# zhangzhousuper/Radish_PT

Hardware: AMD Instinct MI355X
Metric: Mrays/s (higher is better)
Workload: dtype f32

## Files before the change

### radish_pt_amd/_build.py

```python
import os
import subprocess
import sys

ROOT = os.path.dirname(os.path.dirname(os.path.abspath(__file__)))
CSRC = os.path.join(ROOT, "radish_pt_amd", "csrc")
HIPCC = os.environ.get("HIPCC", "/opt/rocm/bin/hipcc")

HOST_SOURCES = [os.path.join(CSRC, "host", "scene_build.cpp"), os.path.join(CSRC, "host", "scene_load.cpp")]
HIP_SOURCES = [os.path.join(CSRC, "radish_hip.hip")]
HIP_DEPS = [
    os.path.join(CSRC, "device", f)
    for f in ("rmath.h", "layouts.h", "traverse.h", "bsdf.h", "lights.h", "path_step.h", "kernels_pt.h", "kernels_restir.h", "kernels_wave.h", "kernels_persist.h", "kernels_walk.h", "wg_trace.h", "kernels_display.h", "kernels_denoise.h", "kernels_bvh.h", "kernels_refit.h", "kernels_lbvh.h", "kernels_lights.h", "kernels_pose.h", "kernels_materials.h", "kernels_textures.h")
] + [os.path.join(ROOT, "include", "radish_hip.h")]

HIP_FLAGS = [
    "--offload-arch=gfx950", "-O3", "-std=c++17", "-fPIC", "-shared", "-ffp-contract=off", "-fno-fast-math",
    "-fno-gpu-rdc", "-Wall", "-Wno-unused-function", "-Wno-unused-value", "-Wno-unused-result",
]


def _newer(target, deps):
    if not os.path.exists(target):
        return True
    t = os.path.getmtime(target)
    return any(os.path.exists(d) and os.path.getmtime(d) > t for d in deps)


def _run(cmd):
    print("[build]", " ".join(cmd), flush=True)
    subprocess.check_call(cmd)


def build_host(force=False):
    out = os.path.join(CSRC, "libradish_host.so")
    deps = HOST_SOURCES + [os.path.join(ROOT, "include", "radish_host.h")]
    if force or _newer(out, deps):
        _run(["g++", "-O2", "-std=c++17", "-fPIC", "-shared", "-ffp-contract=off", "-fno-fast-math", "-Wall", "-o", out]
             + HOST_SOURCES + ["-lz"])
    return out


def build_hip(force=False):
    out = os.path.join(CSRC, "libradish_hip.so")
    if force or _newer(out, HIP_SOURCES + HIP_DEPS):
        _run([HIPCC] + HIP_FLAGS + ["-I", os.path.join(ROOT, "include"), "-o", out] + HIP_SOURCES
             + ["-Wl,-rpath,/opt/rocm/lib"])
    return out


def build_variant(name, defines):
    d = os.path.join(CSRC, "variants")
    os.makedirs(d, exist_ok=True)
    out = os.path.join(d, f"libradish_hip_{name}.so")
    _run([HIPCC] + HIP_FLAGS + [f"-D{x}" for x in defines] + ["-I", os.path.join(ROOT, "include"), "-o", out]
         + HIP_SOURCES + ["-Wl,-rpath,/opt/rocm/lib"])
    return out


def build_all(force=False):
    build_host(force)
    build_hip(force)


if __name__ == "__main__":
    build_all(force="--force" in sys.argv)
```

### radish_pt_amd/csrc/device/kernels_wave.h

```cpp
#pragma once
#include "kernels_pt.h"
#include "wg_trace.h"

namespace rd {

constexpr int kWfLitCap = 8192;
constexpr int kWfLitShadow = 0x40000000;
constexpr int kMaxWaveDepth = 32;

struct alignas(128) WaveCounter {
    int v;
    int pad[31];
};
#ifndef RD_WF_TICKET_SHARDS
#define RD_WF_TICKET_SHARDS 8
#endif
constexpr int kTicketShards = RD_WF_TICKET_SHARDS;
struct WaveCounters {
    WaveCounter rayCount[kMaxWaveDepth + 2];
    WaveCounter shadowCount[kMaxWaveDepth + 2];
    WaveCounter litCount[kMaxWaveDepth + 2];
    WaveCounter traceHead[kMaxWaveDepth + 2];
    WaveCounter shadeHead[kMaxWaveDepth + 2][4];
    WaveCounter traceTicket[kMaxWaveDepth + 2][kTicketShards];
    WaveCounter shadeTicket[kMaxWaveDepth + 2][kTicketShards];
};

struct WaveWorkspace {
    float4 *ro[2];
    float4 *rd[2];
    float4 *thr[2];
    float4 *prevPos[2];
    float4 *accD;
    float4 *accI;
    float4 *nee[2];
    float4 *sht[2];
    uint2 *rng[2];
    int4 *hit;
    int *rayq[2];
    int *shadowq;
    int *litq[2];
    int litCap;
    int *treeOvf;
    int treeOvfDepth;
#ifdef RD_WF_STAMPS
    unsigned long long *stamps;
    int stampWaves;
#endif
    WaveCounters *ctr;
};

constexpr unsigned kWfNeeNone = 2u;
RD_DEV float wfNeeTag(int home, unsigned kind) { return __uint_as_float(((unsigned)home << 2) | kind); }
RD_DEV void wfAddNee(const WaveWorkspace &w, float4 n) {
    const unsigned tag = __float_as_uint(n.w), kind = tag & 3u;
    if (kind == kWfNeeNone) return;
    float4 *acc = (kind == 0u ? w.accD : w.accI) + (tag >> 2);
    const float4 a = *acc;
    *acc = make_float4(a.x + n.x, a.y + n.y, a.z + n.z, 0.f);
}

RD_DEV Ray wfSlotRay(const WaveWorkspace &w, int set, int p, bool shadow, float &limit) {
    if (shadow) {
        const float4 x = w.prevPos[set][p], y = w.sht[set][p];
        return shadowRay(mk3(x.x, x.y, x.z), mk3(y.x, y.y, y.z), limit);
    }
    const float4 o = w.ro[set][p], d = w.rd[set][p];
    limit = 3.402823466e+38f;
    return Ray{mk3(o.x, o.y, o.z), mk3(d.x, d.y, d.z)};
}

struct WaveSlotPath {
    const WaveWorkspace &w;
    const int rs, p;
    const int wr, q;
    int home;
    const bool delta;
    RD_DEV v3 throughput() {
        const float4 t = w.thr[rs][p];
        home = __float_as_int(t.w);
        return mk3(t.x, t.y, t.z);
    }
    RD_DEV float samplePdf() const { return w.ro[rs][p].w; }
    RD_DEV bool sampleDelta() const { return delta; }
    RD_DEV v3 prevPos() const { const float4 c = w.prevPos[rs][p]; return mk3(c.x, c.y, c.z); }
    RD_DEV void setDirect(v3 v) { w.accD[home] = make_float4(v.x, v.y, v.z, 0.f); }
    RD_DEV void addIndirect(v3 v) { const float4 a = w.accI[home]; w.accI[home] = make_float4(a.x + v.x, a.y + v.y, a.z + v.z, 0.f); }
    RD_DEV Sampler rng(const DScene &s) const { const uint2 r = w.rng[rs][p]; return Sampler{s.sobol, r.x, (int)r.y}; }
    RD_DEV void setNee(v3 c, float nw) { w.nee[wr][q] = make_float4(c.x, c.y, c.z, wfNeeTag(home, nw < 0.f ? kWfNeeNone : (nw == 0.f ? 0u : 1u))); }
    RD_DEV void setPrevPos(v3 x) { w.prevPos[wr][q] = make_float4(x.x, x.y, x.z, 0.f); }
    RD_DEV void setRay(const Ray &ray, float pdf, bool deltaSample, v3 throughput, const Sampler &rng) {
        w.ro[wr][q] = make_float4(ray.o.x, ray.o.y, ray.o.z, pdf);
        w.rd[wr][q] = make_float4(ray.d.x, ray.d.y, ray.d.z, deltaSample ? 1.f : 0.f);
        w.thr[wr][q] = make_float4(throughput.x, throughput.y, throughput.z, __int_as_float(home));
        w.rng[wr][q] = make_uint2(rng.scramble, (unsigned)rng.ptr);
    }
};


RD_DEV void waveAppend(bool pred, int item, int *queue, int *count) {
    unsigned long long mask = __ballot(pred);
    if (mask == 0ull) return;
    int leader = __ffsll((long long)mask) - 1;
    int base = 0;
    if ((int)(threadIdx.x & 63u) == leader) base = atomicAdd(count, __popcll(mask));
    base = __shfl(base, leader, 64);
    if (pred) queue[base + __popcll(mask & laneMaskLt())] = item;
}

constexpr int kShadeChunks = 4;
constexpr int kShadePacket = 64 * kShadeChunks;
RD_DEV void waveAppendN(const bool (&pred)[kShadeChunks], const int (&item)[kShadeChunks], int *queue, int *count) {
    unsigned long long m[kShadeChunks];
    int total = 0;
#pragma unroll
    for (int j = 0; j < kShadeChunks; j++) {
        m[j] = __ballot(pred[j]);
        total += __popcll(m[j]);
    }
    if (total == 0) return;
    int base = 0;
    if ((threadIdx.x & 63u) == 0u) base = atomicAdd(count, total);
    base = __shfl(base, 0, 64);
#pragma unroll
    for (int j = 0; j < kShadeChunks; j++) {
        if (pred[j]) queue[base + __popcll(m[j] & laneMaskLt())] = item[j];
        base += __popcll(m[j]);
    }
}

constexpr int kPacket = 128;
RD_DEV int gridWaves() { return int(gridDim.x * (blockDim.x >> 6)); }
RD_DEV int workgroupTicket(WaveCounter *tickets) {
    __shared__ int ticket;
    if (threadIdx.x == 0) {
        const unsigned x = blockIdx.x % (unsigned)kTicketShards;
        ticket = int(x + (unsigned)kTicketShards * (unsigned)atomicAdd(&tickets[x].v, 1));
    }
    __syncthreads();
    return __builtin_amdgcn_readfirstlane(ticket);
}
RD_DEV int logicalWave(int wg) { return __builtin_amdgcn_readfirstlane(int(wg * int(blockDim.x >> 6) + int(threadIdx.x >> 6))); }
RD_DEV int wavePull(int *head, int packet = kPacket) {
    int base = 0;
    if ((threadIdx.x & 63u) == 0u) base = atomicAdd(head, packet);
    return __shfl(base, 0, 64) + gridWaves() * packet;
}

RD_DEV unsigned subFrameBlocks(const PixelMap &pm, int part, int parts) { return (unsigned)(pm.numBlocks - part + parts - 1) / (unsigned)parts; }
constexpr int kSobolRows = 10000;
__global__ __launch_bounds__(256) void k_wf_raygen(DScene s, DCamera cam, PixelMap pm, WaveWorkspace w, int looper, int samples, int part,
                                                   int parts) {
    unsigned wg;
    const unsigned nLocal = subFrameBlocks(pm, part, parts);
    const unsigned nGroups = nLocal * (unsigned)samples;
    bool wgValid = xcdSwizzle(blockIdx.x, (nGroups + 3u) >> 2, wg);
    unsigned lane = threadIdx.x & 63u;
    unsigned group = wgValid ? wg * 4u + (threadIdx.x >> 6) : 0xffffffffu / 64u;
    const bool inRange = wgValid && group < nGroups;
    const unsigned b = group / nLocal, blockLocal = group - b * nLocal;
    Pix px = mapPixel(pm, inRange ? blockLocal * (unsigned)parts + (unsigned)part : 0xffffffffu / 64u, lane);
    bool valid = px.valid && inRange;
    int p = int(group * 64u + lane);
    bool listed = false;
    if (valid) {
        Sampler rng = makeSeededRandomEngine(int(((unsigned)looper + b) % (unsigned)kSobolRows), px.index, 0, s.sobol);
        Ray ray = cameraSample(cam, px.x, px.y, sample4D(rng));
        w.ro[0][p] = make_float4(ray.o.x, ray.o.y, ray.o.z, 0.f);
        w.rd[0][p] = make_float4(ray.d.x, ray.d.y, ray.d.z, 0.f);
        w.accD[p] = make_float4(0.f, 0.f, 0.f, 0.f);
        w.accI[p] = make_float4(0.f, 0.f, 0.f, 0.f);
        w.rng[0][p] = make_uint2(rng.scramble, (unsigned)rng.ptr);
        if (fabs_(ray.d.x) < 1.1e-6f || fabs_(ray.d.y) < 1.1e-6f || fabs_(ray.d.z) < 1.1e-6f) {
            const int at = atomicAdd(&w.ctr->litCount[0].v, 1);
            if (at < w.litCap) {
                w.litq[0][at] = p;
                listed = true;
            }
        }
    }
    if (inRange) w.rayq[0][p] = valid ? (listed ? -2 - p : p) : -1;
    if (blockIdx.x == 0 && threadIdx.x == 0) w.ctr->rayCount[0].v = int(nGroups) * 64;
}

#ifndef RD_REFILL_MIN
#define RD_REFILL_MIN 16
#endif
#ifndef RD_WF_FINISH_MIN
#define RD_WF_FINISH_MIN 16
#endif
#ifndef RD_WF_SHADOW_FIRST
#define RD_WF_SHADOW_FIRST 0
#endif
constexpr int kWfStampKinds = 3;
#ifdef RD_WF_STAMPS
#define RD_WF_STAMP(kind) do { if (stampAt && (threadIdx.x & 63u) == 0u) stampAt[kind] = wall_clock64(); } while (0)
#define RD_WF_STAMP_DRY() do { if (exhausted && !stampedDry) { stampedDry = true; RD_WF_STAMP(1); } } while (0)
#else
#define RD_WF_STAMP(kind) ((void)0)
#define RD_WF_STAMP_DRY() ((void)0)
#endif
#ifndef RD_WF_COOP_LONE
#define RD_WF_COOP_LONE 1
#endif

#ifndef RD_WF_TRACE_WAVES
#define RD_WF_TRACE_WAVES 7
#endif
#ifndef RD_WF_PAIR_WAVES
#define RD_WF_PAIR_WAVES 1
#endif
template <bool COUNT, bool PAIRS = false>
__global__ __launch_bounds__(256, PAIRS && !COUNT ? RD_WF_PAIR_WAVES : (!COUNT ? RD_WF_TRACE_WAVES : 1)) void k_wf_trace(DScene s, WaveWorkspace w, int k) {
    WaveCounters *c = w.ctr;
    const int wg = workgroupTicket(c->traceTicket[k]);
#ifdef RD_WF_STAMPS
    unsigned long long *const stampAt = w.stamps ? w.stamps + ((size_t)k * (size_t)w.stampWaves + (size_t)logicalWave(wg)) * kWfStampKinds : nullptr;
    bool stampedDry = false;
    RD_WF_STAMP(0);
#endif
    const int nShadow = (k > 0) ? c->shadowCount[k - 1].v : 0;
    const int nRay = c->rayCount[k].v;
    const int total = nShadow + nRay;
    const int *rayq = w.rayq[k & 1];
    const int set = k & 1;
    WalkStats ws{0, 0};
    unsigned nClosest = 0, nAny = 0, nHits = 0;
    const int end = s.bvhSize;
    const int END = end;

    int resNext = logicalWave(wg) * kPacket, resEnd = resNext + kPacket;
    bool exhausted = resNext >= total;
    if (resEnd > total) resEnd = total;
    RD_WF_STAMP_DRY();

    bool alive = false;
    bool isShadow = false;
    int p = -1;
    RaySlab rs;
    rs.o = rs.d = rs.inv = mk3(0.f);
    rs.cls = 0;
    const NodeRec *nodes = s.nodes[0];
    int ord = 0, cur = kPairNone;
    PairStack sp{0, 0};
    int node = END, pending = -1;
    float tmax = 0.f;
    int hitPrim = -1;
    v2 hitBary = mk2(0.f, 0.f);
    bool occluded = false;

    constexpr int kStackEntries = PAIRS ? 4 * kPairLds * 64 : 1;
    __shared__ union WfTraceLds {
        WgTraceSharedT<256> wg;
        int2 stack[kStackEntries];
    } lds;
    WgTraceSharedT<256> &wgsh = lds.wg;
    int2 *const stk = lds.stack + (PAIRS ? int(threadIdx.x >> 6) * kPairLds * 64 : 0);
    int2 *const ovf = PAIRS ? reinterpret_cast<int2 *>(w.treeOvf) + (size_t)logicalWave(wg) * (size_t)w.treeOvfDepth * 64 : nullptr;
    const int nLit = c->litCount[k].v < w.litCap ? c->litCount[k].v : w.litCap;
    for (int it = wg; it < nLit; it += int(gridDim.x)) {
        const int e = w.litq[k & 1][it];
        const bool sh = (e & kWfLitShadow) != 0;
        const int pp = e & (kWfLitShadow - 1);
        float lim;
        const Ray ray = wfSlotRay(w, set, pp, sh, lim);
        const RaySlab urs = makeRaySlab(ray);
        if (urs.cls == 0 || end == 0) continue;
        const NodeRec *un = s.nodes[getMTBVHId(-ray.d)];
        const CoopTrace ct = sh ? wgTraceWhole<true, 256>(s, un, urs, lim, wgsh) : wgTraceWhole<false, 256>(s, un, urs, lim, wgsh);
        if (threadIdx.x == 0) {
            if (sh) {
                nAny++;
                if (!ct.found) wfAddNee(w, w.nee[set][pp]);
            } else {
                nClosest++;
                const bool hit = ct.hitPrim != -1;
                if (hit) nHits++;
                w.hit[pp] = make_int4(ct.hitPrim, __float_as_int(hit ? ct.bary.x : 0.f), __float_as_int(hit ? ct.bary.y : 0.f),
                                      hit ? int(s.primClass[ct.hitPrim]) : 0);
            }
            if (COUNT) {
                ws.nodes += ct.nodes;
                ws.tris += ct.tris;
            }
        }
    }
    if (PAIRS) __syncthreads();
    bool firstRound = true;
    bool fromList = false;
    for (;;) {
        bool doStart = false;
        fromList = false;
        if (firstRound) {
            firstRound = false;
            const int it = wg + (int(threadIdx.x & 63u) * 4 + int(threadIdx.x >> 6)) * int(gridDim.x);
            if (it < nLit) {
                const int e = w.litq[k & 1][it];
                doStart = true;
                fromList = true;
                isShadow = (e & kWfLitShadow) != 0;
                p = e & (kWfLitShadow - 1);
            }
        }
        unsigned long long idle = __ballot(!alive && !doStart && p < 0);
        int nIdle = __popcll(idle);
        if (!exhausted && nIdle >= RD_REFILL_MIN) {
            int myRank = __popcll(idle & laneMaskLt());
            int taken = 0;
            while (taken < nIdle && !exhausted) {
                if (resNext == resEnd) {
                    resNext = wavePull(&c->traceHead[k].v);
                    resEnd = resNext + kPacket;
                    if (resNext >= total) {
                        exhausted = true;
                        break;
                    }
                    if (resEnd > total) resEnd = total;
                }
                int avail = resEnd - resNext;
                int give = (nIdle - taken) < avail ? (nIdle - taken) : avail;
                if (!alive && !doStart && p < 0 && myRank >= taken && myRank < taken + give) {
                    const int item = resNext + (myRank - taken);
                    doStart = true;
#if RD_WF_SHADOW_FIRST
                    isShadow = item < nShadow;
                    p = isShadow ? w.shadowq[item] : rayq[item - nShadow];
#else
                    isShadow = item >= nRay;
                    p = isShadow ? w.shadowq[item - nRay] : rayq[item];
#endif
                }
                resNext += give;
                taken += give;
            }
        }
        RD_WF_STAMP_DRY();
        if (doStart) {
            if (p >= 0) {
                const Ray ray = wfSlotRay(w, set, p, isShadow, tmax);
                if (isShadow) nAny++;
                else nClosest++;
                rs = makeRaySlab(ray);
                pending = -1;
                if (PAIRS) {
                    ord = getMTBVHId(-ray.d);
                    sp = PairStack{0, 0};
                    if (rs.cls == 0 || end == 0) pairStart<COUNT>(s, rs, tmax, cur, pending, ws);
                    else cur = kPairFresh;
                    alive = true;
                } else {
                    nodes = s.nodes[getMTBVHId(-ray.d)];
                    node = 0;
                    alive = node != END;
                }
                hitPrim = -1;
                occluded = false;
                if (fromList && rs.cls != 0 && end != 0) {
                    if (isShadow) nAny--;
                    else nClosest--;
                    alive = false;
                    p = -1;
                }
            }
        }
        unsigned long long am = __ballot(alive);
        if (am == 0ull) {
            if (exhausted) break;
            continue;
        }

        {
            unsigned long long lit = __ballot(PAIRS ? (alive && cur == kPairFresh) : (alive && rs.cls != 0 && node == 0 && pending < 0));
            while (lit) {
                const int L = __ffsll((long long)lit) - 1;
                lit &= lit - 1ull;
                const bool shadowL = readlaneI(isShadow ? 1 : 0, L) != 0;
                const NodeRec *un = PAIRS ? s.nodes[0] + (size_t)readlaneI(ord, L) * (size_t)(end + 1) : readlanePtr(nodes, L);
                const RaySlab ur = readlaneRay(rs, L);
                const float lim = readlaneF(tmax, L);
                CoopTrace ct = shadowL ? coopTraceWhole<true>(s, un, ur, lim) : coopTraceWhole<false>(s, un, ur, lim);
                if (int(threadIdx.x & 63u) == L) {
                    hitPrim = ct.hitPrim;
                    hitBary = ct.bary;
                    tmax = ct.tmax;
                    occluded = ct.found;
                    node = END;
                    cur = kPairNone;
                    alive = false;
                    if (COUNT) {
                        ws.nodes += ct.nodes;
                        ws.tris += ct.tris;
                    }
                }
            }
        }
        if (PAIRS) {
            bool busy = alive && pending < 0;
            const int nStart = __popcll(__ballot(busy));
            if (nStart > 0) {
                const int minWalk = (nStart * (RD_LEAF_DEN - RD_LEAF_NUM) + RD_LEAF_DEN - 1) / RD_LEAF_DEN;
                const int lane = int(threadIdx.x & 63u);
                do {
                    pairPopOne<COUNT>(stk, lane, ovf, tmax, busy, cur, sp, pending, ws);
                    if (busy && cur >= 0) {
                        pairStep<COUNT>(s.pairs, stk, lane, ovf, rs, tmax, ord, cur, sp, pending, ws);
                        busy = pending < 0 && (cur >= 0 || sp.sp > 0);
                    }
                } while (__popcll(__ballot(busy)) >= (minWalk > 1 ? minWalk : 1));
                alive = alive && (pending >= 0 || cur >= 0 || sp.sp > 0);
            }
        } else
        {
            bool walking = alive && pending < 0;
            const int nStart = __popcll(__ballot(walking));
#if RD_WF_COOP_LONE
            if (nStart == 1) {
                const int L = __ffsll((long long)__ballot(walking)) - 1;
                CoopResult cr = coopWalk(readlanePtr(nodes, L), readlaneI(node, L), end, readlaneRay(rs, L), readlaneF(tmax, L), RD_COOP_WINDOWS);
                if (int(threadIdx.x & 63u) == L) {
                    node = cr.node;
                    pending = cr.pending;
                    if (COUNT) ws.nodes += cr.visited;
                    alive = (node != end) || pending >= 0;
                }
            } else
#endif
            if (nStart > 0) {
                const int minWalk = (nStart * (RD_LEAF_DEN - RD_LEAF_NUM) + RD_LEAF_DEN - 1) / RD_LEAF_DEN;
                do {
                    if (walking) {
                        if (COUNT) ws.nodes++;
                        float4 lo = nodes[node].lo_prim;
                        float4 hi = nodes[node].hi_next;
                        float boundDist;
                        bool boundHit = aabbFast(lo, hi, rs, boundDist);
                        if (boundHit && boundDist < tmax) {
                            pending = __float_as_int(lo.w);
                            node++;
                        } else {
                            node = __float_as_int(hi.w);
                        }
                        walking = pending < 0 && node != END;
                        alive = (node != END) || pending >= 0;
                    }
                } while (__popcll(__ballot(walking)) >= (minWalk > 1 ? minWalk : 1));
            }
        }
        if (alive && pending >= 0) {
            TriVerts t = loadTri(s.tris, pending);
            float dist;
            v2 bary;
            if (COUNT) ws.tris++;
            bool hit = intersectTriangle(rs, t.a, t.b, t.c, bary, dist);
            if (hit && dist < tmax) {
                if (isShadow) {
                    occluded = true;
                    node = END;
                    cur = kPairNone;
                    sp = PairStack{0, 0};
                } else {
                    hitPrim = pending;
                    tmax = dist;
                    hitBary = bary;
                }
            }
            pending = -1;
            alive = PAIRS ? (cur >= 0 || sp.sp > 0) : (node != END);
        }
        const unsigned long long doneM = __ballot(!alive && p >= 0);
// ... 172 lines not shown
```

### radish_pt_amd/csrc/radish_hip.hip

```cpp
#include "radish_hip.h"

#include <hip/hip_runtime.h>
#include <dlfcn.h>

#include <algorithm>
#include <cfloat>
#include <climits>
#include <cmath>
#include <cstdarg>
#include <cstdio>
#include <cstring>
#include <mutex>
#include <string>
#include <type_traits>
#include <utility>
#include <vector>

#include "device/kernels_pt.h"
#include "device/kernels_restir.h"
#include "device/kernels_wave.h"
#include "device/kernels_persist.h"
#include "device/kernels_walk.h"
#include "device/kernels_display.h"
#include "device/kernels_denoise.h"
// ... 522 lines not shown
    pm.world = c->world;
    pm.tilesPerRank = (pm.numTiles + pm.world - 1) / pm.world;
    pm.packed = (c->world > 1 || c->forcePacked) ? 1 : 0;
    int bpe = pm.tile / 8;
    pm.numBlocks = pm.tilesPerRank * bpe * bpe;
    return pm;
}

constexpr int kPairMinNodes = 0;
bool usePairs(const rdh_ctx *c, uint32_t flags) {
    if (!c->scene.ds.pairs || (flags & RDH_PT_NO_PAIRS)) return false;
    if (flags & RDH_PT_PAIRS) return true;
    if (c->pairMode >= 0) return c->pairMode != 0;
    return c->scene.ds.bvhSize >= kPairMinNodes;
}

bool usePackets(uint32_t flags) {
    static const int env = getenv("RADISH_PACKETS") ? atoi(getenv("RADISH_PACKETS")) : 1;
    return env != 0 && !(flags & RDH_PT_NO_PACKETS);
}

unsigned gridFor(const PixelMap &pm) {
    unsigned work = (unsigned)(pm.numBlocks + 3) / 4;
    return ((work + 7u) / 8u) * 8u;
}

unsigned gridBlocks(const PixelMap &pm) { return (((unsigned)pm.numBlocks + 7u) / 8u) * 8u; }

int settleTree(rdh_ctx *c) {
    if (!c->scene.treePending) return RDH_OK;
    HIP_TRY(c, hipEventSynchronize(c->evTree));
    c->scene.treePending = false;
    if (c->scene.treeRefit) {
        c->scene.treeRefit = false;
        if (!c->scene.ds.pairs) return RDH_OK;
        const int4 lo = c->hTreeHdr.as<int4>()[1], hi = c->hTreeHdr.as<int4>()[2];
        c->scene.ds.rootLo = make_float4(__builtin_bit_cast(float, lo.x), __builtin_bit_cast(float, lo.y), __builtin_bit_cast(float, lo.z), c->scene.ds.rootLo.w);
        c->scene.ds.rootHi = make_float4(__builtin_bit_cast(float, hi.x), __builtin_bit_cast(float, hi.y), __builtin_bit_cast(float, hi.z), c->scene.ds.rootHi.w);
        return RDH_OK;
    }
    const int4 *hdr = c->hTreeHdr.as<int4>(), h0 = hdr[0], lo = hdr[1], hi = hdr[2];
    if (h0.y != 0) {
        c->scene.haveScene = false;
        return fail(c, RDH_ERR_STATE, "device BVH build failed (error bits %d); the scene must be uploaded again", h0.y);
    }
    constexpr int kMaxPairDepth = 2048;
    const PairRec *pairs = c->scene.updPairs ? c->scene.updPairs : c->scene.ds.pairs;
    if (h0.x <= kMaxPairDepth) {
        c->scene.ds.pairs = pairs;
        c->scene.ds.treeDepth = h0.x;
        c->scene.ds.rootLo = make_float4(__builtin_bit_cast(float, lo.x), __builtin_bit_cast(float, lo.y), __builtin_bit_cast(float, lo.z),
                                   __builtin_bit_cast(float, lo.w));
        c->scene.ds.rootHi = make_float4(__builtin_bit_cast(float, hi.x), __builtin_bit_cast(float, hi.y), __builtin_bit_cast(float, hi.z),
                                   __builtin_bit_cast(float, hi.w));
    } else {
        c->scene.ds.pairs = nullptr;
        c->scene.ds.treeDepth = 0;
    }
    return RDH_OK;
}

int settleLights(rdh_ctx *c) {
    if (!c->scene.lightsPending) return RDH_OK;
    HIP_TRY(c, hipEventSynchronize(c->evLights));
    c->scene.lightsPending = false;
    c->scene.ds.sumLightPowerInv = c->hLightSums.as<float>()[1];
    return RDH_OK;
}

int requireReady(rdh_ctx *c) {
    if (!c) return RDH_ERR_ARGS;
    if (c->scene.haveScene) {
        int rc = settleTree(c);
        if (rc) return rc;
        if ((rc = settleLights(c))) return rc;
    }
    if (!c->scene.haveScene) return fail(c, RDH_ERR_NO_SCENE, "no scene uploaded (rdh_scene_upload)");
    if (!c->haveCamera) return fail(c, RDH_ERR_NO_SCENE, "no camera set (rdh_set_camera)");
    return RDH_OK;
}

constexpr size_t kProfilePairs = 8192;

long profBegin(rdh_ctx *c, uint32_t flags) {
    if (!(flags & RDH_PT_PROFILE) || c->profUsed >= kProfilePairs) return -1;
    if (c->profEvents.size() < 2 * (c->profUsed + 1)) {
        hipEvent_t a = nullptr, b = nullptr;
        if (newEvent(c, &a, true) || newEvent(c, &b, true)) return -1;
        c->profEvents.push_back(a);
        c->profEvents.push_back(b);
    }
    long i = (long)c->profUsed++;
    hipEventRecord(c->profEvents[2 * i], c->stream);
    return i;
}
void profEnd(rdh_ctx *c, long i) {
    if (i >= 0) hipEventRecord(c->profEvents[2 * i + 1], c->stream);
}

constexpr unsigned kPersistentGrid = 256u * 8u;

template <typename T>
int wfAlloc(rdh_ctx *c, T **out, size_t count) {
    void *p = nullptr;
    HIP_TRY(c, hipMalloc(&p, std::max<size_t>(count * sizeof(T), 16)));
    c->wfAllocs.push_back(p);
    *out = static_cast<T *>(p);
    return RDH_OK;
}

int wavefrontEnsure(rdh_ctx *c, const PixelMap &pm, int samples) {
    long long slots = (long long)pm.numBlocks * 64 * samples;
    if (c->wfCapacity >= slots) return RDH_OK;
    for (void *p : c->wfAllocs) hipFree(p);
    c->wfAllocs.clear();
    c->wfCapacity = 0;
    const size_t n0 = (size_t)slots, n1 = (size_t)((slots / 64 + 1) / 2) * 64;
    for (int h = 0; h < kWfParts; h++) {
        WaveWorkspace &w = c->wf[h];
        const size_t n = h == 0 ? n0 : n1;
        int rc = RDH_OK;
        for (int set = 0; set < 2 && rc == RDH_OK; set++) {
            if ((rc = wfAlloc(c, &w.ro[set], n)) || (rc = wfAlloc(c, &w.rd[set], n)) || (rc = wfAlloc(c, &w.thr[set], n)) ||
                (rc = wfAlloc(c, &w.prevPos[set], n)) || (rc = wfAlloc(c, &w.nee[set], n)) || (rc = wfAlloc(c, &w.sht[set], n)) ||
                (rc = wfAlloc(c, &w.rng[set], n)))
                return rc;
        }
        if ((rc = wfAlloc(c, &w.accD, n)) || (rc = wfAlloc(c, &w.accI, n)) ||
            (rc = wfAlloc(c, &w.hit, n)) || (rc = wfAlloc(c, &w.rayq[0], n)) || (rc = wfAlloc(c, &w.rayq[1], n)) ||
            (rc = wfAlloc(c, &w.shadowq, n)) || (rc = wfAlloc(c, &w.ctr, 1)) || (rc = wfAlloc(c, &w.litq[0], (size_t)kWfLitCap)) ||
            (rc = wfAlloc(c, &w.litq[1], (size_t)kWfLitCap)))
            return rc;
        w.litCap = 0;
    }
    if (!c->evWfFork) {
        int rc;
        if ((rc = newEvent(c, &c->evWfFork)) || (rc = newEvent(c, &c->evWfJoin))) return rc;
        HIP_TRY(c, hipStreamCreateWithFlags(&c->wfStream, hipStreamNonBlocking));
        if ((rc = newEvent(c, &c->evWfJoin3))) return rc;
    }
    c->wfCapacity = slots;
    return RDH_OK;
}

int wavefrontPathTrace(rdh_ctx *c, const PixelMap &pm, float *d_direct, float *d_indirect, int iter, int looper, int samples,
                       int maxDepth, uint32_t flags) {
    if (maxDepth > kMaxWaveDepth) return fail(c, RDH_ERR_ARGS, "maxDepth %d exceeds %d", maxDepth, kMaxWaveDepth);
    const bool count = (flags & RDH_PT_COUNT) != 0, sort = (flags & RDH_PT_SORT_MATERIAL) != 0;
    const bool tree = usePairs(c, flags);
    unsigned traceRes = 0, shadeRes = 0;
    int rq = RDH_OK;
    withBools([&](auto cnt, auto pr) { rq = residentGrid(c, k_wf_trace<cnt.value, pr.value>, 256, &traceRes); }, count, tree);
    if (rq || (rq = residentGrid(c, k_wf_shade, 256, &shadeRes))) return rq;
    const unsigned traceGrid = sharedGrid(c, std::min(traceRes, kPersistentGrid), kUnbounded);
    const unsigned shadeGrid = sharedGrid(c, std::min(shadeRes, kPersistentGrid), kUnbounded);
    static const int partsEnv = getenv("RADISH_WF_PARTS") ? atoi(getenv("RADISH_WF_PARTS")) : kWfPartsDefault;
    int parts = ((flags & RDH_PT_WF_SUBFRAMES) && pm.numBlocks >= 2048) ? (partsEnv >= 1 && partsEnv <= kWfParts ? partsEnv : kWfPartsDefault) : 1;
    const int ovfDepth = c->scene.ds.treeDepth + 1;
    const size_t ovfNeed = (size_t)traceGrid * 4 * 64 * (size_t)ovfDepth * 2;
    if (tree && parts > 1 && (size_t)parts * ovfNeed * sizeof(int) > kWfStripBudget) parts = 1;
    hipStream_t sts[kWfParts] = {c->stream, c->sideStream, c->wfStream};
    if (tree) {
        for (int h = 0; h < parts; h++) {
            if (int rc = grow(c, c->wfTreeOvf[h], ovfNeed, ovfNeed * sizeof(int), Busy::Device)) return rc;
            c->wf[h].treeOvf = c->wfTreeOvf[h].as<int>();
            c->wf[h].treeOvfDepth = ovfDepth;
        }
    }
#ifdef RD_WF_STAMPS
    {
        const size_t stamps = (size_t)(maxDepth + 1) * traceGrid * 4 * kWfStampKinds;
        if (int rc = grow(c, c->wfStamps, stamps, stamps * sizeof(unsigned long long), Busy::Device)) return rc;
        HIP_TRY(c, hipMemsetAsync(c->wfStamps.p, 0, stamps * sizeof(unsigned long long), c->stream));
        for (int h = 0; h < kWfParts; h++) {
            c->wf[h].stamps = h == 0 ? c->wfStamps.as<unsigned long long>() : nullptr;
            c->wf[h].stampWaves = (int)(traceGrid * 4);
        }
        c->wfStampStages = maxDepth + 1;
        c->wfStampWaves = (int)(traceGrid * 4);
    }
#endif
    const long pf = parts >= 2 ? profBegin(c, flags) : -1;
    if (parts >= 2) {
        HIP_TRY(c, hipEventRecord(c->evWfFork, c->stream));
        for (int h = 1; h < parts; h++) HIP_TRY(c, hipStreamWaitEvent(sts[h], c->evWfFork, 0));
    }
    int rc = RDH_OK;
    auto keep = [&](hipError_t e, const char *what) {
        if (e != hipSuccess && rc == RDH_OK) rc = fail(c, (int)e, "HIP error (%s:%d): %s: %s", __FILE__, __LINE__, what, hipGetErrorString(e));
    };
    for (int h = 0; h < parts; h++) {
        const unsigned waves = traceGrid * 4u;
        c->wf[h].litCap = (int)(waves * 64u < (unsigned)kWfLitCap ? waves * 64u : (unsigned)kWfLitCap);
        if (flags & RDH_PT_WF_SMALL_LISTS) c->wf[h].litCap = 4;
    }
    for (int h = 0; h < parts; h++) {
        hipStream_t st = sts[h];
        WaveWorkspace &w = c->wf[h];
        const unsigned nLocal = (unsigned)(pm.numBlocks - h + parts - 1) / (unsigned)parts;
        const unsigned gridBlk = (((nLocal * (unsigned)samples + 3u) / 4u + 7u) / 8u) * 8u;
        keep(hipMemsetAsync(w.ctr, 0, sizeof(WaveCounters), st), "hipMemsetAsync(wavefront counters)");
        hipLaunchKernelGGL(k_wf_raygen, dim3(gridBlk), dim3(256), 0, st, c->scene.ds, c->cam, pm, w, looper, samples, h, parts);
    }
    for (int k = 0; k <= maxDepth && rc == RDH_OK; k++) {
        for (int h = 0; h < parts; h++) {
            hipStream_t st = sts[h];
            WaveWorkspace &w = c->wf[h];
            long pe = (h == 0 && parts == 1) ? profBegin(c, flags) : -1;
            withBools([&](auto cnt, auto pr) {
                hipLaunchKernelGGL((k_wf_trace<cnt.value, pr.value>), dim3(traceGrid), dim3(256), 0, st, c->scene.ds, w, k);
            }, count, tree);
            profEnd(c, pe);
            hipLaunchKernelGGL(k_wf_shade, dim3(shadeGrid), dim3(256), 0, st, c->scene.ds, w, k, maxDepth, sort ? 1 : 0);
        }
        keep(hipGetLastError(), "wavefront stage launch");
    }
    for (int h = 0; h < parts && rc == RDH_OK; h++) {
        hipStream_t st = sts[h];
        const unsigned nLocal = (unsigned)(pm.numBlocks - h + parts - 1) / (unsigned)parts;
        const unsigned gridBlk = (((nLocal + 3u) / 4u + 7u) / 8u) * 8u;
        hipLaunchKernelGGL(k_wf_finish, dim3(gridBlk), dim3(256), 0, st, pm, c->wf[h], iter, samples, d_direct, d_indirect, h, parts);
    }
    keep(hipGetLastError(), "k_wf_finish");
    if (parts >= 2) {
        hipError_t e1 = hipEventRecord(c->evWfJoin, c->sideStream);
        hipError_t e2 = hipStreamWaitEvent(c->stream, c->evWfJoin, 0);
        hipError_t e3 = hipEventRecord(c->evWfJoin3, c->wfStream);
        hipError_t e4 = hipStreamWaitEvent(c->stream, c->evWfJoin3, 0);
        if (e1 != hipSuccess || e2 != hipSuccess || e3 != hipSuccess || e4 != hipSuccess) {
            hipStreamSynchronize(c->sideStream);
            hipStreamSynchronize(c->wfStream);
            keep(e1 != hipSuccess ? e1 : (e2 != hipSuccess ? e2 : (e3 != hipSuccess ? e3 : e4)), "wavefront join");
        }
    }
    profEnd(c, pf);
    return rc;
}

int ensureStackOverflow(rdh_ctx *c, unsigned resident) {
    const size_t ints = (size_t)resident * 64 * (size_t)(c->scene.ds.treeDepth + 1) * 2;
    return grow(c, c->treeOvf, ints, ints * sizeof(int), Busy::Device);
}

uint32_t resolveStructure(const rdh_ctx *c, const PixelMap &pm, uint32_t flags) {
    if (!(flags & RDH_PT_AUTO)) return flags;
    flags &= ~(RDH_PT_AUTO | RDH_PT_WAVEFRONT | RDH_PT_SORT_MATERIAL | RDH_PT_WF_SUBFRAMES | RDH_PT_PERSISTENT);
    const bool wavefront = c->scene.ds.bvhSize >= 100000 && pm.numBlocks >= 12000;
    return flags | (wavefront ? (RDH_PT_WAVEFRONT | RDH_PT_SORT_MATERIAL | RDH_PT_WF_SUBFRAMES) : RDH_PT_PERSISTENT);
}

int packetBudget(uint32_t flags) { return (flags & RDH_PT_WF_SMALL_LISTS) ? 4 : kPacketBudget; }

int launchWalk(rdh_ctx *c, const float *d_rays, long long n, int4 *d_hits, int *d_occ, bool count, const int *deferCount = nullptr,
               const int *deferList = nullptr, int slotList = 0, bool pairs = false, bool packets = false, int budget = kPacketBudget) {
    const bool any = d_occ != nullptr, defer = deferCount != nullptr;
    packets = packets && !any && n > 0 && (n + 255) / 256 <= 0x7fffffffll;
    if (pairs && !c->scene.ds.pairs) return fail(c, RDH_ERR_UNSUPPORTED, "RDH_PT_PAIRS: the uploaded node arrays are not six orderings of one binary tree, or that tree is more than 2 048 levels deep");
    unsigned resGrid = 0;
    int rc = RDH_OK;
    withBools([&](auto a) {
        rc = pairs ? residentGrid(c, k_walk_pair<false, a.value>, 64, &resGrid) : residentGrid(c, k_walk_persistent<false, a.value>, 64, &resGrid);
    }, any);
    if (rc) return rc;
    const unsigned grid = sharedGrid(c, resGrid, (unsigned long long)((n + 63) / 64));
    const int ovfDepth = c->scene.ds.treeDepth + 1;
    if (pairs && !packets && (rc = ensureStackOverflow(c, resGrid))) return rc;
    int2 *const ovf = c->treeOvf.as<int2>();
    if (!packets) HIP_TRY(c, hipMemsetAsync(c->dPersist, 0, offsetof(PersistCounters, deferred), c->stream));
    if (defer) {
        if ((rc = forkLiteral(c))) return rc;
        withBools([&](auto cnt, auto a) {
            hipLaunchKernelGGL((k_trace_wg_list<cnt.value, a.value>), dim3(kWalkDeferCap), dim3(kWgTraceThreads), 0, c->litStream, c->scene.ds, d_rays, deferList, deferCount, d_hits, d_occ);
        }, count, any);
    }
    if (packets) {
        const unsigned pgrid = (unsigned)((n + 255) / 256);
        withBools([&](auto cnt, auto def) {
            hipLaunchKernelGGL((k_walk_packet<cnt.value, def.value>), dim3(pgrid), dim3(256), 0, c->stream, c->scene.ds, d_rays, n, d_hits, deferCount, slotList, budget);
        }, count, defer);
    } else {
        withBools([&](auto cnt, auto a, auto def) {
            if (pairs)
                hipLaunchKernelGGL((k_walk_pair<cnt.value, a.value, def.value>), dim3(grid), dim3(64), 0, c->stream, c->scene.ds, d_rays, n, d_hits, d_occ,
                                   c->dPersist, ovf, ovfDepth, deferCount, slotList);
            else
                hipLaunchKernelGGL((k_walk_persistent<cnt.value, a.value, def.value>), dim3(grid), dim3(64), 0, c->stream, c->scene.ds, d_rays, n, d_hits, d_occ,
                                   c->dPersist, deferCount, slotList);
        }, count, any, defer);
    }
    if (defer) joinLiteral(c);
    HIP_TRY(c, hipGetLastError());
    return RDH_OK;
}

RestirSplit splitLayout(Carver &k, size_t slots) {
    RestirSplit sp;
    sp.st = k.take<float4>(slots * 48);
    sp.hits = k.take<int4>(slots * 16);
    sp.rays = k.take<float>(slots * 24);
    sp.segs = k.take<float>(slots * 24);
    sp.rawResv = k.take<float>(slots * 36);
    sp.occ = k.take<int>(slots * 4);
    sp.deferCount = k.take<int>(16 + 2 * sizeof(int) * kRestirDeferCap);
    sp.deferList = sp.deferCount + 4;
    return sp;
}

void timeBegin(rdh_ctx *c) {
    hipEventRecord(c->evStart, c->stream);
}
int timeEnd(rdh_ctx *c, const char *what) {
    hipEventRecord(c->evStop, c->stream);
    c->timed = true;
    hipError_t e = hipGetLastError();
    if (e != hipSuccess) return fail(c, (int)e, "HIP error: %s: %s", what, hipGetErrorString(e));
    return RDH_OK;
}

}

extern "C" {

int rdh_create(rdh_ctx **out, int device) {
    if (!out) return RDH_ERR_ARGS;
    *out = nullptr;
    int n = 0;
    if (hipGetDeviceCount(&n) != hipSuccess || n <= 0 || device < 0 || device >= n) return RDH_ERR_NO_DEVICE;
    if (hipSetDevice(device) != hipSuccess) return RDH_ERR_NO_DEVICE;
    rdh_ctx *c = new rdh_ctx;
    c->device = device;
    if (hipStreamCreateWithFlags(&c->ownStream, hipStreamNonBlocking) != hipSuccess ||
        newEvent(c, &c->evStart, true) || newEvent(c, &c->evStop, true) ||
        hipStreamCreateWithFlags(&c->sideStream, hipStreamNonBlocking) != hipSuccess ||
        newEvent(c, &c->evFork) || newEvent(c, &c->evJoin) || newEvent(c, &c->evFrame) || newEvent(c, &c->evSched[0]) ||
        newEvent(c, &c->evSched[1]) ||
        hipMalloc((void **)&c->dCounters, sizeof(Counters)) != hipSuccess ||
        hipMalloc((void **)&c->dPersist, sizeof(PersistCounters)) != hipSuccess) {
        delete c;
        return RDH_ERR_NO_DEVICE;
    }
    c->stream = c->ownStream;
    c->litStream = c->sideStream;
    {
        const char *e = getenv("RADISH_LIT_PRIORITY");
        int least = 0, greatest = 0;
        if (e && atoi(e) != 0 && hipDeviceGetStreamPriorityRange(&least, &greatest) == hipSuccess && greatest < least) {
            hipStream_t hs = nullptr;
// ... 2398 lines not shown
```

Measured before the change: 3008.

## Add sharded trace work handout with static slots and cap pair-trace grid

Reworks how k_wf_trace waves obtain ray packets. Each wave now starts from a static slot computed by a new handout helper, then pulls further packets from optionally sharded head counters, stealing from other shards once its own runs dry. The change also replaces launch_bounds with an explicit waves-per-EU range, raises the default pair-traversal occupancy target from 1 to 6, and caps the trace grid at CU count times that target. The aim is less contention on the work-queue atomic and better register/occupancy balance, at the cost of more handout logic and possible load imbalance at the tail.

```diff
diff --git a/radish_pt_amd/_build.py b/radish_pt_amd/_build.py
--- a/radish_pt_amd/_build.py
+++ b/radish_pt_amd/_build.py
@@ -10,7 +10,7 @@
 HIP_SOURCES = [os.path.join(CSRC, "radish_hip.hip")]
 HIP_DEPS = [
     os.path.join(CSRC, "device", f)
-    for f in ("rmath.h", "layouts.h", "traverse.h", "bsdf.h", "lights.h", "path_step.h", "kernels_pt.h", "kernels_restir.h", "kernels_wave.h", "kernels_persist.h", "kernels_walk.h", "wg_trace.h", "kernels_display.h", "kernels_denoise.h", "kernels_bvh.h", "kernels_refit.h", "kernels_lbvh.h", "kernels_lights.h", "kernels_pose.h", "kernels_materials.h", "kernels_textures.h")
+    for f in ("rmath.h", "layouts.h", "traverse.h", "bsdf.h", "lights.h", "path_step.h", "kernels_pt.h", "kernels_restir.h", "kernels_wave.h", "kernels_persist.h", "kernels_walk.h", "wg_trace.h", "wf_handout.h", "kernels_display.h", "kernels_denoise.h", "kernels_bvh.h", "kernels_refit.h", "kernels_lbvh.h", "kernels_lights.h", "kernels_pose.h", "kernels_materials.h", "kernels_textures.h")
 ] + [os.path.join(ROOT, "include", "radish_hip.h")]
 
 HIP_FLAGS = [
diff --git a/radish_pt_amd/csrc/device/kernels_wave.h b/radish_pt_amd/csrc/device/kernels_wave.h
--- a/radish_pt_amd/csrc/device/kernels_wave.h
+++ b/radish_pt_amd/csrc/device/kernels_wave.h
@@ -1,6 +1,7 @@
 #pragma once
 #include "kernels_pt.h"
 #include "wg_trace.h"
+#include "wf_handout.h"
 
 namespace rd {
 
@@ -16,11 +17,16 @@
 #define RD_WF_TICKET_SHARDS 8
 #endif
 constexpr int kTicketShards = RD_WF_TICKET_SHARDS;
+#ifndef RD_WF_HEAD_SHARDS
+#define RD_WF_HEAD_SHARDS 1
+#endif
+constexpr int kHeadShards = RD_WF_HEAD_SHARDS;
+static_assert(kHeadShards >= 1 && kHeadShards <= 8, "the dry mask of k_wf_trace is read from lanes 0 .. kHeadShards - 1");
 struct WaveCounters {
     WaveCounter rayCount[kMaxWaveDepth + 2];
     WaveCounter shadowCount[kMaxWaveDepth + 2];
     WaveCounter litCount[kMaxWaveDepth + 2];
-    WaveCounter traceHead[kMaxWaveDepth + 2];
+    WaveCounter traceHead[kMaxWaveDepth + 2][kHeadShards];
     WaveCounter shadeHead[kMaxWaveDepth + 2][4];
     WaveCounter traceTicket[kMaxWaveDepth + 2][kTicketShards];
     WaveCounter shadeTicket[kMaxWaveDepth + 2][kTicketShards];
@@ -43,6 +49,7 @@
     int litCap;
     int *treeOvf;
     int treeOvfDepth;
+    int ownShards;
 #ifdef RD_WF_STAMPS
     unsigned long long *stamps;
     int stampWaves;
@@ -130,6 +137,16 @@
 }
 
 constexpr int kPacket = 128;
+#ifndef RD_WF_STATIC
+#define RD_WF_STATIC 128
+#endif
+#ifndef RD_WF_PACKET
+#define RD_WF_PACKET 128
+#endif
+#ifndef RD_WF_LIST_NO_STATIC
+#define RD_WF_LIST_NO_STATIC 0
+#endif
+constexpr int kTraceStatic = RD_WF_STATIC, kTracePacket = RD_WF_PACKET;
 RD_DEV int gridWaves() { return int(gridDim.x * (blockDim.x >> 6)); }
 RD_DEV int workgroupTicket(WaveCounter *tickets) {
     __shared__ int ticket;
@@ -145,6 +162,34 @@
     int base = 0;
     if ((threadIdx.x & 63u) == 0u) base = atomicAdd(head, packet);
     return __shfl(base, 0, 64) + gridWaves() * packet;
+}
+RD_DEV int traceListed(const WaveCounters *c, const WaveWorkspace &w, int k) {
+    if (!RD_WF_LIST_NO_STATIC) return 0;
+    const int nLit = c->litCount[k].v < w.litCap ? c->litCount[k].v : w.litCap;
+    return handout::listedWorkgroups(nLit, int(gridDim.x), true);
+}
+RD_DEV int tracePull(WaveCounters *c, const WaveWorkspace &w, int k, unsigned &dry, int total) {
+    WaveCounter *const heads = c->traceHead[k];
+    const int lane = int(threadIdx.x & 63u);
+    const int base = handout::dynBase(int(gridDim.x), int(blockDim.x >> 6), traceListed(c, w, k), kTraceStatic);
+    const int own = handout::ownShard(int(blockIdx.x), kHeadShards, w.ownShards);
+    if (base >= total) return -1;
+    for (;;) {
+        const int x = __builtin_amdgcn_readfirstlane(handout::nextShard(own, dry, kHeadShards));
+        if (x < 0) return -1;
+        int n = 0;
+        if (lane == 0) n = atomicAdd(&heads[x].v, 1);
+        n = __builtin_amdgcn_readfirstlane(n);
+        const int begin = handout::packetBegin(base, handout::pulledPacket(n, x, kHeadShards), kTracePacket);
+        if (begin < total) return begin;
+        dry |= 1u << x;
+        if (kHeadShards > 1) {
+            int seen = 0;
+            if (lane < kHeadShards) seen = __hip_atomic_load(&heads[lane].v, __ATOMIC_RELAXED, __HIP_MEMORY_SCOPE_AGENT);
+            const bool gone = lane < kHeadShards && handout::packetBegin(base, handout::pulledPacket(seen, lane, kHeadShards), kTracePacket) >= total;
+            dry |= (unsigned)__ballot(gone);
+        }
+    }
 }
 
 RD_DEV unsigned subFrameBlocks(const PixelMap &pm, int part, int parts) { return (unsigned)(pm.numBlocks - part + parts - 1) / (unsigned)parts; }
@@ -208,10 +253,12 @@
 #define RD_WF_TRACE_WAVES 7
 #endif
 #ifndef RD_WF_PAIR_WAVES
-#define RD_WF_PAIR_WAVES 1
+#define RD_WF_PAIR_WAVES 6
 #endif
 template <bool COUNT, bool PAIRS = false>
-__global__ __launch_bounds__(256, PAIRS && !COUNT ? RD_WF_PAIR_WAVES : (!COUNT ? RD_WF_TRACE_WAVES : 1)) void k_wf_trace(DScene s, WaveWorkspace w, int k) {
+__global__ __attribute__((amdgpu_flat_work_group_size(1, 256),
+                          amdgpu_waves_per_eu(PAIRS && !COUNT ? RD_WF_PAIR_WAVES : (!COUNT ? RD_WF_TRACE_WAVES : 1),
+                                              PAIRS && !COUNT ? RD_WF_PAIR_WAVES : 8))) void k_wf_trace(DScene s, WaveWorkspace w, int k) {
     WaveCounters *c = w.ctr;
     const int wg = workgroupTicket(c->traceTicket[k]);
 #ifdef RD_WF_STAMPS
@@ -229,9 +276,13 @@
     const int end = s.bvhSize;
     const int END = end;
 
-    int resNext = logicalWave(wg) * kPacket, resEnd = resNext + kPacket;
-    bool exhausted = resNext >= total;
+    const int nLit = c->litCount[k].v < w.litCap ? c->litCount[k].v : w.litCap;
+    const int slot = __builtin_amdgcn_readfirstlane(handout::staticSlot(wg, int(threadIdx.x >> 6), int(blockDim.x >> 6), traceListed(c, w, k)));
+    unsigned dryHeads = 0u;
+    int resNext = slot < 0 ? 0 : slot * kTraceStatic, resEnd = slot < 0 ? 0 : resNext + kTraceStatic;
+    bool exhausted = slot >= 0 && resNext >= total;
     if (resEnd > total) resEnd = total;
+    if (resNext > resEnd) resNext = resEnd;
     RD_WF_STAMP_DRY();
 
     bool alive = false;
@@ -257,7 +308,6 @@
     WgTraceSharedT<256> &wgsh = lds.wg;
     int2 *const stk = lds.stack + (PAIRS ? int(threadIdx.x >> 6) * kPairLds * 64 : 0);
     int2 *const ovf = PAIRS ? reinterpret_cast<int2 *>(w.treeOvf) + (size_t)logicalWave(wg) * (size_t)w.treeOvfDepth * 64 : nullptr;
-    const int nLit = c->litCount[k].v < w.litCap ? c->litCount[k].v : w.litCap;
     for (int it = wg; it < nLit; it += int(gridDim.x)) {
         const int e = w.litq[k & 1][it];
         const bool sh = (e & kWfLitShadow) != 0;
@@ -309,12 +359,13 @@
             int taken = 0;
             while (taken < nIdle && !exhausted) {
                 if (resNext == resEnd) {
-                    resNext = wavePull(&c->traceHead[k].v);
-                    resEnd = resNext + kPacket;
-                    if (resNext >= total) {
+                    resNext = tracePull(c, w, k, dryHeads, total);
+                    if (resNext < 0) {
+                        resNext = resEnd;
                         exhausted = true;
                         break;
                     }
+                    resEnd = resNext + kTracePacket;
                     if (resEnd > total) resEnd = total;
                 }
                 int avail = resEnd - resNext;
diff --git a/radish_pt_amd/csrc/device/wf_handout.h b/radish_pt_amd/csrc/device/wf_handout.h
--- /dev/null
+++ b/radish_pt_amd/csrc/device/wf_handout.h
@@ -0,0 +1,35 @@
+#pragma once
+
+#if defined(__HIPCC__) || defined(__CUDACC__)
+#define RD_HANDOUT_FN __host__ __device__ inline
+#else
+#define RD_HANDOUT_FN inline
+#endif
+
+namespace rd {
+namespace handout {
+
+RD_HANDOUT_FN int listedWorkgroups(int nLit, int grid, bool skipListed) { return skipListed ? (nLit < grid ? nLit : grid) : 0; }
+
+RD_HANDOUT_FN int staticSlot(int wg, int wave, int wavesPerWg, int listed) { return wg < listed ? -1 : (wg - listed) * wavesPerWg + wave; }
+
+RD_HANDOUT_FN int dynBase(int grid, int wavesPerWg, int listed, int staticItems) { return (grid - listed) * wavesPerWg * staticItems; }
+
+RD_HANDOUT_FN int pulledPacket(int n, int shard, int shards) { return n * shards + shard; }
+
+RD_HANDOUT_FN int packetBegin(int base, int j, int packetItems) { return base + j * packetItems; }
+
+RD_HANDOUT_FN int ownShard(int block, int shards, int ownShards) { return (block % shards) % ownShards; }
+
+RD_HANDOUT_FN int stealShard(int own, int i, int shards) { return (own + i) % shards; }
+
+RD_HANDOUT_FN int nextShard(int own, unsigned dryMask, int shards) {
+    for (int i = 0; i < shards; i++) {
+        const int x = stealShard(own, i, shards);
+        if (!((dryMask >> x) & 1u)) return x;
+    }
+    return -1;
+}
+
+}
+}
diff --git a/radish_pt_amd/csrc/radish_hip.hip b/radish_pt_amd/csrc/radish_hip.hip
--- a/radish_pt_amd/csrc/radish_hip.hip
+++ b/radish_pt_amd/csrc/radish_hip.hip
@@ -698,6 +698,11 @@
     int rq = RDH_OK;
     withBools([&](auto cnt, auto pr) { rq = residentGrid(c, k_wf_trace<cnt.value, pr.value>, 256, &traceRes); }, count, tree);
     if (rq || (rq = residentGrid(c, k_wf_shade, 256, &shadeRes))) return rq;
+    if (tree && !count) {
+        int cus = 0;
+        if (int rc = cuCount(c, &cus)) return rc;
+        traceRes = std::min(traceRes, (unsigned)cus * (unsigned)RD_WF_PAIR_WAVES);
+    }
     const unsigned traceGrid = sharedGrid(c, std::min(traceRes, kPersistentGrid), kUnbounded);
     const unsigned shadeGrid = sharedGrid(c, std::min(shadeRes, kPersistentGrid), kUnbounded);
     static const int partsEnv = getenv("RADISH_WF_PARTS") ? atoi(getenv("RADISH_WF_PARTS")) : kWfPartsDefault;
@@ -739,6 +744,7 @@
         const unsigned waves = traceGrid * 4u;
         c->wf[h].litCap = (int)(waves * 64u < (unsigned)kWfLitCap ? waves * 64u : (unsigned)kWfLitCap);
         if (flags & RDH_PT_WF_SMALL_LISTS) c->wf[h].litCap = 4;
+        c->wf[h].ownShards = (flags & RDH_PT_WF_SMALL_LISTS) ? 1 : kHeadShards;
     }
     for (int h = 0; h < parts; h++) {
         hipStream_t st = sts[h];
```

Result: no change. 3013 (median of 3 runs) (+0.2%).
